# yoshitomo-matsubara/hnd-ghnd-object-detectors

Measured on AMD Instinct MI355X. Metric: distill-step images/sec at 3x800x1333, GHND Faster R-CNN b3ch, higher is better.
Workload: dtype f32

## Files before the change

hnd_ghnd_object_detectors_amd/csrc/conv_bx3.hip:

```cpp

#include "bf16x3.h"
#include "common.h"

#include <stdlib.h>

namespace {

using hnd::bf8;
using hnd::cu_count;
using hnd::f32x4;
using hnd::FastDiv;
using hnd::split_pair;
using hnd::static_for;
using hnd::u32x4;

struct Bx3Args {
  FastDiv div_ow, div_oh;
  int nsl;
  int nchunks;
  int mrows;
  int cpg;
  int res_up;
};

template <int OFF>
__device__ __forceinline__ void rload(f32x4& dst, const float* p) {
  asm volatile("global_load_dwordx4 %0, %1, off offset:%2" : "=a"(dst) : "v"(p), "n"(OFF));
}
template <int CNT>
__device__ __forceinline__ void rwait(f32x4& a0, f32x4& a1, f32x4& a2, f32x4& a3, f32x4& a4, f32x4& a5, f32x4& a6,
                                      f32x4& a7) {
  asm volatile("s_waitcnt vmcnt(%8)"
               : "+a"(a0), "+a"(a1), "+a"(a2), "+a"(a3), "+a"(a4), "+a"(a5), "+a"(a6), "+a"(a7)
               : "n"(CNT));
}

__device__ __forceinline__ void bload(uint32_t& dst, const uint8_t* p) {
  asm volatile("global_load_ubyte %0, %1, off" : "=a"(dst) : "v"(p));
}
template <int CNT>
__device__ __forceinline__ void bwait8(uint32_t& a0, uint32_t& a1, uint32_t& a2, uint32_t& a3, uint32_t& a4, uint32_t& a5,
                                       uint32_t& a6, uint32_t& a7) {
  asm volatile("s_waitcnt vmcnt(%8)"
               : "+a"(a0), "+a"(a1), "+a"(a2), "+a"(a3), "+a"(a4), "+a"(a5), "+a"(a6), "+a"(a7)
               : "n"(CNT));
}

template <int CNT>
__device__ __forceinline__ void rwait8(f32x4& a0, f32x4& a1, f32x4& a2, f32x4& a3, f32x4& a4, f32x4& a5, f32x4& a6,
                                       f32x4& a7) {
  rwait<CNT>(a0, a1, a2, a3, a4, a5, a6, a7);
}

template <int KS, bool RES, bool MO, bool MK = false>
__global__ void __launch_bounds__(256, 1) bx3_kernel(const hnd_conv_desc d, const Bx3Args a) {
  static_assert(!MK || RES, "the mask build rides on the residual build's bookkeeping");
  constexpr int RESLOADS = RES ? (MK ? 32 : 16) : 0;
  constexpr int RING = RES ? 2 : 4, K = 32 * KS, MI = 4, NI = 4, PLANE = 64 * K, STORES = MO ? 32 : 16;
  static_assert(KS % RING == 0, "ring slots are compile-time: the ring must divide the k steps of a tile");
  extern __shared__ __attribute__((aligned(16))) uint16_t Bs[];
  const int tid = threadIdx.x, lane = tid & 63, wave = tid >> 6;
  const int l16 = lane & 15, g4 = lane >> 4;
  const int b = blockIdx.x, xcd = b & 7, idx = b >> 3, per_xcd = gridDim.x >> 3;
  const int slice = idx % a.nsl, tpx = per_xcd / a.nsl;
  const int team = xcd * tpx + idx / a.nsl, nteams = 8 * tpx;
  const int n0 = slice * 64;
  const int c_lo = (int)((long long)a.nchunks * team / nteams);
  const int c_hi = (int)((long long)a.nchunks * (team + 1) / nteams);

  auto a_ptr = [&](int cc, int mi) -> const float* {
    const unsigned m = min((unsigned)(cc * 64 + mi * 16 + l16), (unsigned)(a.mrows - 1));
    const unsigned t = hnd::fdiv(m, a.div_ow), ow_ = m - t * (unsigned)d.ow;
    const unsigned n_ = hnd::fdiv(t, a.div_oh), oh_ = t - n_ * (unsigned)d.oh;
    const size_t pix = ((size_t)n_ * d.h + oh_ * (unsigned)d.sh) * (size_t)d.w_ + ow_ * (unsigned)d.sw;
    return d.x + pix * (size_t)d.cin + (size_t)(g4 * 8);
  };
  const int col0 = n0 + l16 * 4;
  float es[NI], eb[NI];
#pragma unroll
  for (int ni = 0; ni < NI; ++ni) {
    es[ni] = d.epi_scale ? d.epi_scale[col0 + ni] : 1.f;
    eb[ni] = d.epi_shift ? d.epi_shift[col0 + ni] : 0.f;
  }
  const size_t slice_elems = (size_t)3 * PLANE;

  int c = c_lo;
  while (c < c_hi) {
    const int grp = a.cpg > 0 ? c / a.cpg : 0;
    const int seg_hi = a.cpg > 0 ? min(c_hi, (grp + 1) * a.cpg) : c_hi;
    __syncthreads();
    {
      const u32x4* src = (const u32x4*)(d.w_bf16x3 + ((size_t)grp * a.nsl + slice) * slice_elems);
      u32x4* dst = (u32x4*)Bs;
      constexpr int NV = 3 * PLANE / 8, UB = 12;
      static_assert(NV % (256 * UB) == 0, "slice does not divide among the threads");
#pragma unroll 1
      for (int i0 = 0; i0 < NV; i0 += 256 * UB) {
        u32x4 t[UB];
#pragma unroll
        for (int u = 0; u < UB; ++u) t[u] = src[i0 + u * 256 + tid];
#pragma unroll
        for (int u = 0; u < UB; ++u) dst[i0 + u * 256 + tid] = t[u];
      }
    }
    __syncthreads();

    int cc = c + wave;
    if (cc < seg_hi) {
      const float* aptr[MI];
      f32x4 ring[RING][MI][2];
#pragma unroll
      for (int mi = 0; mi < MI; ++mi) aptr[mi] = a_ptr(cc, mi);
      static_for<RING>([&](auto U) __attribute__((always_inline)) {
        constexpr int u = decltype(U)::value;
        static_for<MI>([&](auto I) __attribute__((always_inline)) {
          constexpr int mi = decltype(I)::value;
          rload<(u % KS) * 128>(ring[u][mi][0], aptr[mi]);
          rload<(u % KS) * 128 + 16>(ring[u][mi][1], aptr[mi]);
        });
      });
      uint32_t pl[2][3][MI][4];
      float dummy = 0.f;
#pragma unroll
      for (int i = 0; i < STORES; ++i) asm volatile("global_load_dword %0, %1, off" : "+v"(dummy) : "v"(aptr[0]));
      rwait<8 * (RING - 1) + STORES>(ring[0][0][0], ring[0][0][1], ring[0][1][0], ring[0][1][1], ring[0][2][0], ring[0][2][1],
                                     ring[0][3][0], ring[0][3][1]);
#pragma unroll
      for (int mi = 0; mi < MI; ++mi)
#pragma unroll
        for (int j = 0; j < 4; ++j) {
          const f32x4 v = ring[0][mi][j >> 1];
          const float x0 = (j & 1) ? v.z : v.x, x1 = (j & 1) ? v.w : v.y;
          split_pair(x0, x1, pl[0][0][mi][j], pl[0][1][mi][j], pl[0][2][mi][j]);
        }
      f32x4 acc[MI][NI];
      bf8 bfirst[3];
      {
        const uint16_t* br = Bs + l16 * K + ((g4 ^ l16) * 8);
        bfirst[0] = *(const bf8*)(br); bfirst[1] = *(const bf8*)(br + PLANE); bfirst[2] = *(const bf8*)(br + 2 * PLANE);
      }
      f32x4 resv[MI][4];
      uint32_t resm[MI][4];
      for (; cc < seg_hi; cc += 4) {
        const int cn = cc + 4 < seg_hi ? cc + 4 : cc;
        const float* nptr[MI];
#pragma unroll
        for (int mi = 0; mi < MI; ++mi) nptr[mi] = a_ptr(cn, mi);
        static_for<KS>([&](auto G) __attribute__((always_inline)) {
          constexpr int ks = decltype(G)::value, slot = ks % RING, par = ks & 1;
          constexpr int slot1 = (ks + 1) % RING;
          if constexpr (MK && ks == KS - 4) {
#pragma unroll
            for (int mi = 0; mi < MI; ++mi)
#pragma unroll
              for (int r = 0; r < 4; ++r)
                bload(resm[mi][r], d.mask_bits + (((size_t)min(cc * 64 + mi * 16 + g4 * 4 + r, a.mrows - 1) * (size_t)d.ldc + col0) >> 2));
          }
          if constexpr (RES && ks == KS - 4) {
#pragma unroll
            for (int mi = 0; mi < MI; ++mi) {
              const unsigned mr = (unsigned)(cc * 64 + mi * 16 + g4 * 4);
              const unsigned m0 = min(mr, (unsigned)(a.mrows - 4));
              const unsigned t = hnd::fdiv(m0, a.div_ow), ow_ = m0 - t * (unsigned)d.ow;
              const unsigned n_ = hnd::fdiv(t, a.div_oh), oh_ = t - n_ * (unsigned)d.oh;
              const size_t pu = ((size_t)n_ * d.res1_h + (oh_ >> 1)) * (size_t)d.res1_w + (ow_ >> 1);
              const bool up = a.res_up != 0;
              const unsigned ml = (unsigned)(a.mrows - 1);
              const size_t p0 = up ? pu : (size_t)min(mr, ml), p1 = up ? pu : (size_t)min(mr + 1, ml),
                           p2 = up ? pu + 1 : (size_t)min(mr + 2, ml), p3 = up ? pu + 1 : (size_t)min(mr + 3, ml);
              rload<0>(resv[mi][0], d.res1 + p0 * (size_t)d.ldc + col0);
              rload<0>(resv[mi][1], d.res1 + p1 * (size_t)d.ldc + col0);
              rload<0>(resv[mi][2], d.res1 + p2 * (size_t)d.ldc + col0);
              rload<0>(resv[mi][3], d.res1 + p3 * (size_t)d.ldc + col0);
            }
          }
          static_for<MI>([&](auto I) __attribute__((always_inline)) {
            constexpr int mi = decltype(I)::value;
            if constexpr (ks + RING < KS) {
              rload<(ks + RING) * 128>(ring[slot][mi][0], aptr[mi]);
              rload<(ks + RING) * 128 + 16>(ring[slot][mi][1], aptr[mi]);
            } else {
              rload<(ks + RING - KS) * 128>(ring[slot][mi][0], nptr[mi]);
              rload<(ks + RING - KS) * 128 + 16>(ring[slot][mi][1], nptr[mi]);
            }
          });
          constexpr int kResYounger = (RES && ks >= KS - 4 && ks <= KS - 4 + RING - 2) ? RESLOADS : 0;
          if constexpr (ks < RING - 1) {
            rwait<(8 * (RING - 1) + STORES + kResYounger < 63 ? 8 * (RING - 1) + STORES + kResYounger : 63)>(
                ring[slot1][0][0], ring[slot1][0][1], ring[slot1][1][0], ring[slot1][1][1], ring[slot1][2][0],
                ring[slot1][2][1], ring[slot1][3][0], ring[slot1][3][1]);
          } else {
            rwait<8 * (RING - 1) + kResYounger>(ring[slot1][0][0], ring[slot1][0][1], ring[slot1][1][0], ring[slot1][1][1],
                                                ring[slot1][2][0], ring[slot1][2][1], ring[slot1][3][0], ring[slot1][3][1]);
          }
          const int pos = ((ks * 4 + g4) ^ l16) * 8;
          bf8 bcur[3], bnxt[3];
          bcur[0] = bfirst[0]; bcur[1] = bfirst[1]; bcur[2] = bfirst[2];
          static_for<NI>([&](auto NIc) __attribute__((always_inline)) {
            constexpr int ni = decltype(NIc)::value;
            if constexpr (ni + 1 < NI) {
              const uint16_t* br = Bs + ((ni + 1) * 16 + l16) * K + pos;
              bnxt[0] = *(const bf8*)(br); bnxt[1] = *(const bf8*)(br + PLANE); bnxt[2] = *(const bf8*)(br + 2 * PLANE);
            } else {
              const uint16_t* br = Bs + l16 * K + ((((ks + 1) % KS) * 4 + g4) ^ l16) * 8;
              bfirst[0] = *(const bf8*)(br); bfirst[1] = *(const bf8*)(br + PLANE); bfirst[2] = *(const bf8*)(br + 2 * PLANE);
            }
            static_for<MI>([&](auto MIc) __attribute__((always_inline)) {
              constexpr int mi = decltype(MIc)::value;
              auto frag = [&](int q) __attribute__((always_inline)) {
                const u32x4 t = {pl[par][q][mi][0], pl[par][q][mi][1], pl[par][q][mi][2], pl[par][q][mi][3]};
                return __builtin_bit_cast(bf8, t);
              };
              const bf8 ah = frag(0), am = frag(1), al = frag(2);
              constexpr int p = ni * 4 + mi, rg = p >> 2, j = p & 3;
              const f32x4 v = ring[slot1][rg][j >> 1];
              const float x0 = (j & 1) ? v.z : v.x, x1 = (j & 1) ? v.w : v.y;
              f32x4 cacc = (ks == 0) ? f32x4{0.f, 0.f, 0.f, 0.f} : acc[mi][ni];
              cacc = __builtin_amdgcn_mfma_f32_16x16x32_bf16(al, bcur[0], cacc, 0, 0, 0);
              const uint32_t h0 = __float_as_uint(x0) & 0xffff0000u, h1 = __float_as_uint(x1) & 0xffff0000u;
              __builtin_amdgcn_sched_barrier(0);
              cacc = __builtin_amdgcn_mfma_f32_16x16x32_bf16(ah, bcur[2], cacc, 0, 0, 0);
              const float r0 = x0 - __uint_as_float(h0), r1 = x1 - __uint_as_float(h1);
              __builtin_amdgcn_sched_barrier(0);
              cacc = __builtin_amdgcn_mfma_f32_16x16x32_bf16(am, bcur[1], cacc, 0, 0, 0);
              const uint32_t m0 = __float_as_uint(r0) & 0xffff0000u, m1 = __float_as_uint(r1) & 0xffff0000u;
              __builtin_amdgcn_sched_barrier(0);
              cacc = __builtin_amdgcn_mfma_f32_16x16x32_bf16(am, bcur[0], cacc, 0, 0, 0);
              const float q0 = r0 - __uint_as_float(m0), q1 = r1 - __uint_as_float(m1);
              __builtin_amdgcn_sched_barrier(0);
              cacc = __builtin_amdgcn_mfma_f32_16x16x32_bf16(ah, bcur[1], cacc, 0, 0, 0);
              pl[par ^ 1][0][rg][j] = __builtin_amdgcn_perm(h1, h0, 0x07060302u);
              pl[par ^ 1][1][rg][j] = __builtin_amdgcn_perm(m1, m0, 0x07060302u);
              pl[par ^ 1][2][rg][j] = __builtin_amdgcn_perm(__float_as_uint(q1), __float_as_uint(q0), 0x07060302u);
              __builtin_amdgcn_sched_barrier(0);
              cacc = __builtin_amdgcn_mfma_f32_16x16x32_bf16(ah, bcur[0], cacc, 0, 0, 0);
              acc[mi][ni] = cacc;
              __builtin_amdgcn_sched_barrier(0);
            });
            if constexpr (ni + 1 < NI) { bcur[0] = bnxt[0]; bcur[1] = bnxt[1]; bcur[2] = bnxt[2]; }
          });
        });
        if constexpr (RES) {
          rwait8<32>(resv[0][0], resv[0][1], resv[0][2], resv[0][3], resv[1][0], resv[1][1], resv[1][2], resv[1][3]);
          rwait8<32>(resv[2][0], resv[2][1], resv[2][2], resv[2][3], resv[3][0], resv[3][1], resv[3][2], resv[3][3]);
          if constexpr (MK) {
            bwait8<32>(resm[0][0], resm[0][1], resm[0][2], resm[0][3], resm[1][0], resm[1][1], resm[1][2], resm[1][3]);
            bwait8<32>(resm[2][0], resm[2][1], resm[2][2], resm[2][3], resm[3][0], resm[3][1], resm[3][2], resm[3][3]);
          }
        }
#pragma unroll
        for (int mi = 0; mi < MI; ++mi)
#pragma unroll
          for (int r = 0; r < 4; ++r) {
            const size_t m = (size_t)min(cc * 64 + mi * 16 + g4 * 4 + r, a.mrows - 1);
            f32x4 v;
#pragma unroll
            for (int ni = 0; ni < NI; ++ni) {
              float x = acc[mi][ni][r] * es[ni] + eb[ni];
              if (RES) x += resv[mi][r][ni];
              if (MK) x = ((resm[mi][r] >> ni) & 1u) ? x : 0.f;
              v[ni] = d.relu ? fmaxf(x, 0.f) : x;
            }
            const size_t yo = m * (size_t)d.ldc + col0;
            *(f32x4*)(d.y + yo) = v;
            if (MO)
              d.mask_out[yo >> 2] = (uint8_t)((v[0] > 0.f ? 1 : 0) | (v[1] > 0.f ? 2 : 0) | (v[2] > 0.f ? 4 : 0) |
                                              (v[3] > 0.f ? 8 : 0));
          }
#pragma unroll
        for (int mi = 0; mi < MI; ++mi) aptr[mi] = nptr[mi];
      }
      asm volatile("s_waitcnt vmcnt(0)" : "+v"(dummy)::"memory");
    }
    c = seg_hi;
  }
}

__global__ void pack_bx3_kernel(const float* __restrict__ w, uint16_t* __restrict__ img, int rows_pad, int K, int KI, int groups,
                                long long group_stride, long long total) {
  const int nsl = rows_pad / 64;
  const size_t plane = (size_t)64 * KI;
  for (long long e = blockIdx.x * (long long)blockDim.x + threadIdx.x; e < total; e += (long long)gridDim.x * blockDim.x) {
    const int k = (int)(e % K);
    long long t = e / K;
    const int row = (int)(t % rows_pad), g = (int)(t / rows_pad);
    const float x = w[(size_t)g * (size_t)group_stride + (size_t)row * K + k];
    const uint32_t xb = __float_as_uint(x), hb = xb & 0xffff0000u;
    const float r1 = x - __uint_as_float(hb);
    const uint32_t mb = __float_as_uint(r1) & 0xffff0000u;
    const float r2 = r1 - __uint_as_float(mb);
    const int part = k / KI, kk = k - part * KI;
    const int s = row / 64, r = row % 64, c = kk >> 3, pos = c ^ (r & 15);
    uint16_t* o = img + (((size_t)part * groups + g) * nsl + s) * 3 * plane + (size_t)r * KI + pos * 8 + (kk & 7);
    o[0] = (uint16_t)(hb >> 16);
    o[plane] = (uint16_t)(mb >> 16);
    o[2 * plane] = (uint16_t)(__float_as_uint(r2) >> 16);
  }
}

template <int KS, bool RES, bool MO, bool MK = false>
int launch_bx3_t(const hnd_conv_desc& d, const Bx3Args& a, int grid, hipStream_t stream) {
  const size_t lds = (size_t)3 * 64 * 32 * KS * sizeof(uint16_t);
  return hnd::launch_big_lds<bx3_kernel<KS, RES, MO, MK>>(dim3(grid), dim3(256), lds, 160 * 1024, stream, "hnd_conv2d_igemm(bx3)",
                                                          d, a);
}

}

namespace hnd {

static bool bx3_recommended(long long rows_per_image, int kdim, int cout) {
  if (rows_per_image <= 0 || cout <= 0 || cout % 64 != 0) return false;
  if (kdim != 128 && (kdim % 256 != 0 || kdim > 2048)) return false;
  const long long nteams = team_count(cout, 64);
  if (nteams == 0) return false;
  const long long chunks_at_16 = (rows_per_image * 16 + 63) / 64;
  return chunks_at_16 / nteams >= (kdim > 512 ? 16 : 8);
}

bool bx3_applies(const hnd_conv_desc& d) {
  if (!d.w_bf16x3) return false;
  if (d.kh != 1 || d.kw != 1 || d.bh != 0 || d.bw != 0 || d.cin != d.kdim) return false;
  if (d.kdim != 128 && (d.kdim % 256 != 0 || d.kdim > 2048)) return false;
  if (d.stats || d.pro_scale || d.res2 || d.mask || d.bwd_x) return false;
  if (d.mask_bits && d.mask_out) return false;
  if (d.mask_bits && d.kdim <= 256 && (!d.res1 || d.res1_mode != 0)) return false;
  if (d.res1 && ((uintptr_t)d.res1 % 16) != 0) return false;
  if (d.res1 && d.res1_mode == 1 && (d.yh != 2 * d.res1_h || d.yw != 2 * d.res1_w || d.ow % 4 != 0)) return false;
  if (d.cout % 64 != 0 || d.ldc % 4 != 0 || ((uintptr_t)d.y % 16) != 0) return false;
  if (team_count(d.cout, 64) == 0) return false;
  if (d.y_sh != 1 || d.y_sw != 1 || d.y_oh != 0 || d.y_ow != 0 || d.yh != d.oh || d.yw != d.ow) return false;
  if (!samples_inside(d)) return false;
  const long long M = gemm_rows(d);
  if (M < 64 || d.w_group_rows % 64 != 0) return false;
  if (M % 64 != 0 && d.w_group_rows != 0) return false;
  return true;
}

static int launch_bx3_one(const hnd_conv_desc& d, int kpart, hipStream_t stream) {
  Bx3Args a;
  a.div_ow = make_fastdiv((unsigned)d.ow);
  a.div_oh = make_fastdiv((unsigned)d.oh);
  a.nsl = d.cout / 64;
  a.mrows = (int)gemm_rows(d);
  a.nchunks = (a.mrows + 63) / 64;
  a.cpg = d.w_group_rows / 64;
  a.res_up = d.res1 && d.res1_mode == 1;
  const int grid = (cu_count() / 8) * 8;
  if (d.mask_bits)
    return kpart == 128 ? launch_bx3_t<4, true, false, true>(d, a, grid, stream)
                        : launch_bx3_t<8, true, false, true>(d, a, grid, stream);
  const int sel = (kpart == 128 ? 0 : 4) | (d.res1 ? 2 : 0) | (d.mask_out ? 1 : 0);
  switch (sel) {
    case 0: return launch_bx3_t<4, false, false>(d, a, grid, stream);
    case 1: return launch_bx3_t<4, false, true>(d, a, grid, stream);
    case 2: return launch_bx3_t<4, true, false>(d, a, grid, stream);
    case 3: return launch_bx3_t<4, true, true>(d, a, grid, stream);
    case 4: return launch_bx3_t<8, false, false>(d, a, grid, stream);
    case 5: return launch_bx3_t<8, false, true>(d, a, grid, stream);
    case 6: return launch_bx3_t<8, true, false>(d, a, grid, stream);
    default: return launch_bx3_t<8, true, true>(d, a, grid, stream);
  }
}

int launch_bx3_tiled(const hnd_conv_desc& d, int mi, hipStream_t stream);

static const int BX3_TILED_BELOW_K128 = 3, BX3_TILED_BELOW_K256 = 3, BX3_TILED_BELOW_K512 = 10, BX3_TILED_BELOW_KLONG = 16;
static const int BX3_TILED_128_ROWS_FROM = 10;

int bx3_build(const hnd_conv_desc& d) {
  const long long chunks = (gemm_rows(d) + 63) / 64, nteams = team_count(d.cout, 64);
  const long long per_team = (chunks + nteams - 1) / nteams;
  const bool is_long = d.kdim >= 1024;
  const int rows = is_long && per_team >= BX3_TILED_128_ROWS_FROM ? 2 : 1;
  const int forced = debug_picker("bx3_tiled");
  if (forced >= 0) {
    const int mi = debug_picker("bx3_tiled_mi");
    return forced ? (mi == 1 || mi == 2 ? mi : rows) : 0;
  }
  if (d.w_group_rows > 0) return 0;
  const int below = d.kdim <= 128 ? BX3_TILED_BELOW_K128
                                  : (d.kdim <= 256 ? BX3_TILED_BELOW_K256 : (is_long ? BX3_TILED_BELOW_KLONG : BX3_TILED_BELOW_K512));
  return per_team < below ? rows : 0;
}

int launch_bx3(const hnd_conv_desc& d, int build, hipStream_t stream) {
  if (build) return launch_bx3_tiled(d, build, stream);
  if (d.kdim <= 256) return launch_bx3_one(d, d.kdim, stream);
  const long long groups = d.w_group_rows > 0 ? gemm_rows(d) / d.w_group_rows : 1;
  const int parts = d.kdim / 256;
  const size_t part_elems = (size_t)groups * (size_t)(d.cout / 64) * (size_t)3 * 64 * 256;
  for (int p = 0; p < parts; ++p) {
    hnd_conv_desc q = d;
    if (p + 1 < parts) {
      q.relu = 0;
      q.mask_out = nullptr;
      q.mask_bits = nullptr;
    }
    if (p > 0) {
      q.x = d.x + (size_t)256 * p;
      q.w_bf16x3 = d.w_bf16x3 + part_elems * (size_t)p;
      q.epi_shift = nullptr;
      q.res1 = d.y;
      q.res1_mode = 0;
    }
    const int rc = launch_bx3_one(q, 256, stream);
    if (rc) return rc;
  }
  return 0;
}

}

extern "C" int hnd_bf16x3_recommended(int64_t rows_per_image, int kdim, int cout) {
  return hnd::bx3_recommended((long long)rows_per_image, kdim, cout) ? 1 : 0;
}

extern "C" size_t hnd_pack_bf16x3_elems(int rows_pad, int kdim, int groups) {
  if (rows_pad <= 0 || rows_pad % 64 != 0 || kdim <= 0 || kdim % 8 != 0 || groups < 1) return 0;
  return (size_t)groups * (size_t)rows_pad * (size_t)kdim * 3;
}

extern "C" int hnd_pack_bf16x3(const float* w_packed, uint16_t* img, int rows_pad, int kdim, int groups,
                               int64_t group_stride, void* stream) {
  HND_REQUIRE(w_packed && img && rows_pad > 0 && rows_pad % 64 == 0 && (kdim == 128 || (kdim % 256 == 0 && kdim <= 2048)) &&
                  groups >= 1 && (groups == 1 || group_stride >= (int64_t)rows_pad * kdim),
              "hnd_pack_bf16x3: bad arguments (kdim must be 128 or a multiple of 256 up to 2048)");
  const long long total = (long long)groups * rows_pad * kdim;
  long long blocks = (total + 255) / 256;
  if (blocks > 8192) blocks = 8192;
  hipLaunchKernelGGL(pack_bx3_kernel, dim3((unsigned)blocks), dim3(256), 0, hnd::as_stream(stream), w_packed, img, rows_pad,
                     kdim, kdim > 256 ? 256 : kdim, groups, (long long)group_stride, total);
  return hnd::check_launch("hnd_pack_bf16x3");
}
```

Measured before the change: 213.9.

## Add multi-workgroup-per-CU bf16x3 kernel for K=128 1x1 convs with picker

Adds a specialized K=128 1x1 conv kernel that launches 2-3 workgroups per CU and splits each 64-row chunk across the four waves. Loads of activation rows are software-prefetched one k-step ahead. A per-class table, together with a chunk-count limit, decides when the new kernel replaces the existing one. The goal is better occupancy and latency hiding on the small-K GEMMs, at the cost of more code paths and extra weight-tile reloads per workgroup.

New measurement: 214.1 (median of 3 runs). About the same (+0.1%).

```diff
diff --git a/hnd_ghnd_object_detectors_amd/csrc/conv_bx3.hip b/hnd_ghnd_object_detectors_amd/csrc/conv_bx3.hip
--- a/hnd_ghnd_object_detectors_amd/csrc/conv_bx3.hip
+++ b/hnd_ghnd_object_detectors_amd/csrc/conv_bx3.hip
@@ -337,7 +337,26 @@
   return true;
 }
 
+int launch_bx3_k128(const hnd_conv_desc& d, hipStream_t stream);
+
+enum Bx3K128Class { K128_PLAIN, K128_GROUPED, K128_RES, K128_RES_MASK_OUT, K128_RES_MASK_BITS, K128_RES_UP, K128_CLASSES };
+static const bool BX3_K128_WINS[K128_CLASSES] = {true, true, false, false, false, true};
+static const long long BX3_K128_MAX_CHUNKS = 1050;
+
+static bool bx3_k128_wins(const hnd_conv_desc& d) {
+  const int forced = debug_picker("bx3_k128");
+  if (forced >= 0) return forced != 0;
+  const Bx3K128Class cls = d.w_group_rows > 0 ? K128_GROUPED
+                           : !d.res1          ? K128_PLAIN
+                           : d.res1_mode == 1 ? K128_RES_UP
+                           : d.mask_bits      ? K128_RES_MASK_BITS
+                           : d.mask_out       ? K128_RES_MASK_OUT
+                                              : K128_RES;
+  return BX3_K128_WINS[cls] && (gemm_rows(d) + 63) / 64 <= BX3_K128_MAX_CHUNKS;
+}
+
 static int launch_bx3_one(const hnd_conv_desc& d, int kpart, hipStream_t stream) {
+  if (kpart == 128 && bx3_k128_wins(d)) return launch_bx3_k128(d, stream);
   Bx3Args a;
   a.div_ow = make_fastdiv((unsigned)d.ow);
   a.div_oh = make_fastdiv((unsigned)d.oh);
diff --git a/hnd_ghnd_object_detectors_amd/csrc/conv_bx3_k128.hip b/hnd_ghnd_object_detectors_amd/csrc/conv_bx3_k128.hip
--- /dev/null
+++ b/hnd_ghnd_object_detectors_amd/csrc/conv_bx3_k128.hip
@@ -0,0 +1,228 @@
+#include "bf16x3.h"
+#include "common.h"
+
+namespace {
+
+using hnd::bf8;
+using hnd::f32x4;
+using hnd::FastDiv;
+using hnd::static_for;
+using hnd::u32x4;
+
+constexpr int wgs_per_cu(bool mk) { return mk ? 2 : 3; }
+
+struct Bx3mArgs {
+  FastDiv div_ow, div_oh;
+  int nsl;
+  int nchunks;
+  int mrows;
+  int cpg;
+  int res_up;
+};
+
+template <bool RES, bool MO, bool MK>
+__global__ void __launch_bounds__(256, wgs_per_cu(MK)) bx3m_kernel(const hnd_conv_desc d, const Bx3mArgs a) {
+  static_assert(!MK || RES, "mask_bits comes with a residual at K = 128 (bx3_applies)");
+  constexpr int KS = 4, K = 32 * KS, MI = 2, NI = 4, PLANE = 64 * K, R = 16 * MI, UPC = 64 / R;
+  __shared__ __attribute__((aligned(16))) uint16_t Bs[3 * PLANE];
+  const int tid = threadIdx.x, lane = tid & 63, wave = tid >> 6;
+  const int l16 = lane & 15, g4 = lane >> 4;
+  const int b = blockIdx.x, xcd = b & 7, idx = b >> 3, per_xcd = gridDim.x >> 3;
+  const int slice = idx % a.nsl, tpx = per_xcd / a.nsl;
+  const int team = xcd * tpx + idx / a.nsl, nteams = 8 * tpx;
+  const int c_lo = (int)((long long)a.nchunks * team / nteams);
+  const int c_hi = (int)((long long)a.nchunks * (team + 1) / nteams);
+  const int col0 = slice * 64 + l16 * 4;
+  const int mlast = a.mrows - 1;
+
+  auto a_ptr = [&](int row0, int mi) -> const float* {
+    const unsigned m = (unsigned)min(row0 + mi * 16 + l16, mlast);
+    const unsigned t = hnd::fdiv(m, a.div_ow), ow_ = m - t * (unsigned)d.ow;
+    const unsigned n_ = hnd::fdiv(t, a.div_oh), oh_ = t - n_ * (unsigned)d.oh;
+    const size_t pix = ((size_t)n_ * d.h + oh_ * (unsigned)d.sh) * (size_t)d.w_ + ow_ * (unsigned)d.sw;
+    return d.x + pix * (size_t)d.cin + (size_t)(g4 * 8);
+  };
+  float es[NI], eb[NI];
+#pragma unroll
+  for (int ni = 0; ni < NI; ++ni) {
+    es[ni] = d.epi_scale ? d.epi_scale[col0 + ni] : 1.f;
+    eb[ni] = d.epi_shift ? d.epi_shift[col0 + ni] : 0.f;
+  }
+
+  int c = c_lo;
+  while (c < c_hi) {
+    const int grp = a.cpg > 0 ? c / a.cpg : 0;
+    const int seg_hi = a.cpg > 0 ? min(c_hi, (grp + 1) * a.cpg) : c_hi;
+    __syncthreads();
+    {
+      const u32x4* src = (const u32x4*)(d.w_bf16x3 + ((size_t)grp * a.nsl + slice) * (size_t)(3 * PLANE));
+      u32x4* dst = (u32x4*)Bs;
+      constexpr int NV = 3 * PLANE / 8, UB = NV / 256;
+      static_assert(NV % 256 == 0, "slice does not divide among the threads");
+      u32x4 t[UB];
+#pragma unroll
+      for (int u = 0; u < UB; ++u) t[u] = src[u * 256 + tid];
+#pragma unroll
+      for (int u = 0; u < UB; ++u) dst[u * 256 + tid] = t[u];
+    }
+    __syncthreads();
+
+    int u = c * UPC + wave;
+    const int u_hi = min(seg_hi * UPC, (a.mrows + R - 1) / R);
+    if (u < u_hi) {
+      const float* ap[MI];
+      f32x4 raw[MI][2];
+#pragma unroll
+      for (int mi = 0; mi < MI; ++mi) {
+        ap[mi] = a_ptr(u * R, mi);
+        raw[mi][0] = *(const f32x4*)(ap[mi]);
+        raw[mi][1] = *(const f32x4*)(ap[mi] + 4);
+      }
+#pragma unroll 1
+      for (; u < u_hi; u += 4) {
+        const int row0 = u * R;
+        const int un = u + 4 < u_hi ? u + 4 : u;
+        const float* np[MI];
+#pragma unroll
+        for (int mi = 0; mi < MI; ++mi) np[mi] = a_ptr(un * R, mi);
+
+        f32x4 resv[MI][4];
+        uint32_t resm[MI][4];
+        if constexpr (RES) {
+#pragma unroll
+          for (int mi = 0; mi < MI; ++mi) {
+            const int mr = row0 + mi * 16 + g4 * 4;
+            size_t p[4];
+            if (a.res_up) {
+              const unsigned m0 = (unsigned)min(mr, a.mrows - 4);
+              const unsigned t = hnd::fdiv(m0, a.div_ow), ow_ = m0 - t * (unsigned)d.ow;
+              const unsigned n_ = hnd::fdiv(t, a.div_oh), oh_ = t - n_ * (unsigned)d.oh;
+              const size_t pu = ((size_t)n_ * d.res1_h + (oh_ >> 1)) * (size_t)d.res1_w + (ow_ >> 1);
+              p[0] = pu; p[1] = pu; p[2] = pu + 1; p[3] = pu + 1;
+            } else {
+#pragma unroll
+              for (int r = 0; r < 4; ++r) p[r] = (size_t)min(mr + r, mlast);
+            }
+#pragma unroll
+            for (int r = 0; r < 4; ++r) resv[mi][r] = *(const f32x4*)(d.res1 + p[r] * (size_t)d.ldc + col0);
+          }
+        }
+
+        f32x4 acc[MI][NI];
+#pragma unroll
+        for (int mi = 0; mi < MI; ++mi)
+#pragma unroll
+          for (int ni = 0; ni < NI; ++ni) acc[mi][ni] = f32x4{0.f, 0.f, 0.f, 0.f};
+        int boff = l16 * K;
+        asm volatile("" : "+v"(boff));
+        const uint16_t* brow = Bs + boff;
+
+        static_for<KS>([&](auto G) __attribute__((always_inline)) {
+          constexpr int ks = decltype(G)::value;
+          bf8 ah[MI], am[MI], al[MI];
+#pragma unroll
+          for (int mi = 0; mi < MI; ++mi) {
+            u32x4 h, m, l;
+#pragma unroll
+            for (int j = 0; j < 4; ++j) {
+              const f32x4 v = raw[mi][j >> 1];
+              const float x0 = (j & 1) ? v.z : v.x, x1 = (j & 1) ? v.w : v.y;
+              uint32_t hp, mp, lp;
+              hnd::split_pair(x0, x1, hp, mp, lp);
+              h[j] = hp; m[j] = mp; l[j] = lp;
+            }
+            ah[mi] = __builtin_bit_cast(bf8, h);
+            am[mi] = __builtin_bit_cast(bf8, m);
+            al[mi] = __builtin_bit_cast(bf8, l);
+          }
+#pragma unroll
+          for (int mi = 0; mi < MI; ++mi) {
+            const float* q = ks + 1 < KS ? ap[mi] + (ks + 1) * 32 : np[mi];
+            raw[mi][0] = *(const f32x4*)(q);
+            raw[mi][1] = *(const f32x4*)(q + 4);
+          }
+          if constexpr (MK && ks == 0) {
+#pragma unroll
+            for (int mi = 0; mi < MI; ++mi)
+#pragma unroll
+              for (int r = 0; r < 4; ++r)
+                resm[mi][r] = d.mask_bits[((size_t)min(row0 + mi * 16 + g4 * 4 + r, mlast) * (size_t)d.ldc + col0) >> 2];
+          }
+          const int pos = ((ks * 4 + g4) ^ l16) * 8;
+#pragma unroll
+          for (int ni = 0; ni < NI; ++ni) {
+            const uint16_t* br = brow + ni * 16 * K + pos;
+            const bf8 bh = *(const bf8*)(br), bm = *(const bf8*)(br + PLANE), bl = *(const bf8*)(br + 2 * PLANE);
+#pragma unroll
+            for (int mi = 0; mi < MI; ++mi) {
+              f32x4 cacc = acc[mi][ni];
+              cacc = __builtin_amdgcn_mfma_f32_16x16x32_bf16(al[mi], bh, cacc, 0, 0, 0);
+              cacc = __builtin_amdgcn_mfma_f32_16x16x32_bf16(ah[mi], bl, cacc, 0, 0, 0);
+              cacc = __builtin_amdgcn_mfma_f32_16x16x32_bf16(am[mi], bm, cacc, 0, 0, 0);
+              cacc = __builtin_amdgcn_mfma_f32_16x16x32_bf16(am[mi], bh, cacc, 0, 0, 0);
+              cacc = __builtin_amdgcn_mfma_f32_16x16x32_bf16(ah[mi], bm, cacc, 0, 0, 0);
+              cacc = __builtin_amdgcn_mfma_f32_16x16x32_bf16(ah[mi], bh, cacc, 0, 0, 0);
+              acc[mi][ni] = cacc;
+            }
+          }
+        });
+
+#pragma unroll
+        for (int mi = 0; mi < MI; ++mi)
+#pragma unroll
+          for (int r = 0; r < 4; ++r) {
+            const int m = row0 + mi * 16 + g4 * 4 + r;
+            f32x4 v;
+#pragma unroll
+            for (int ni = 0; ni < NI; ++ni) {
+              float x = acc[mi][ni][r] * es[ni] + eb[ni];
+              if (RES) x += resv[mi][r][ni];
+              if (MK) x = ((resm[mi][r] >> ni) & 1u) ? x : 0.f;
+              v[ni] = d.relu ? fmaxf(x, 0.f) : x;
+            }
+            if (m <= mlast) {
+              const size_t yo = (size_t)m * (size_t)d.ldc + col0;
+              *(f32x4*)(d.y + yo) = v;
+              if (MO)
+                d.mask_out[yo >> 2] = (uint8_t)((v[0] > 0.f ? 1 : 0) | (v[1] > 0.f ? 2 : 0) | (v[2] > 0.f ? 4 : 0) |
+                                                (v[3] > 0.f ? 8 : 0));
+            }
+          }
+#pragma unroll
+        for (int mi = 0; mi < MI; ++mi) ap[mi] = np[mi];
+      }
+    }
+    c = seg_hi;
+  }
+}
+
+template <bool RES, bool MO, bool MK>
+int launch_bx3m_t(const hnd_conv_desc& d, const Bx3mArgs& a, hipStream_t stream) {
+  const int grid = wgs_per_cu(MK) * (hnd::cu_count() / 8) * 8;
+  hipLaunchKernelGGL((bx3m_kernel<RES, MO, MK>), dim3(grid), dim3(256), 0, stream, d, a);
+  return hnd::check_launch("hnd_conv2d_igemm(bx3 k128)");
+}
+
+}
+
+namespace hnd {
+
+int launch_bx3_k128(const hnd_conv_desc& d, hipStream_t stream) {
+  Bx3mArgs a;
+  a.div_ow = make_fastdiv((unsigned)d.ow);
+  a.div_oh = make_fastdiv((unsigned)d.oh);
+  a.nsl = d.cout / 64;
+  a.mrows = (int)gemm_rows(d);
+  a.nchunks = (a.mrows + 63) / 64;
+  a.cpg = d.w_group_rows / 64;
+  a.res_up = d.res1 && d.res1_mode == 1;
+  if (d.mask_bits) return launch_bx3m_t<true, false, true>(d, a, stream);
+  switch ((d.res1 ? 2 : 0) | (d.mask_out ? 1 : 0)) {
+    case 0: return launch_bx3m_t<false, false, false>(d, a, stream);
+    case 1: return launch_bx3m_t<false, true, false>(d, a, stream);
+    case 2: return launch_bx3m_t<true, false, false>(d, a, stream);
+    default: return launch_bx3m_t<true, true, false>(d, a, stream);
+  }
+}
+
+}
```
